# folkol/query-engines

Measured on AMD Instinct MI355X. Metric: rows/sec filter+project+group-by over 1B-row Arrow batch; % HBM roofline, higher is better.
Workload: dtype int64; 1 GPU; C4: SELECT k, SUM(a+b), COUNT(*), MIN(a), MAX(b) WHERE a > 2^19 GROUP BY k; rows_per_gpu=1000000000, groups=1024, columns=k, a, b int64 (Arrow, no nulls), parallelism=hash-sharded partial aggregate x1

## Files before the change

query-engines_amd/csrc/qe_dev.hpp:

```cpp
#ifndef QE_DEV_HPP
#define QE_DEV_HPP

#ifndef QE_OP_EQ
#define QE_OP_EQ 10
#define QE_OP_NE 11
#define QE_OP_LT 12
#define QE_OP_LE 13
#define QE_OP_GT 14
#define QE_OP_GE 15
#endif
#ifndef QE_MAX_KEYS
#define QE_MAX_KEYS 4
#define QE_MAX_AGGS 8
#define QE_MAX_COLS 8
#define QE_MAX_TERMS 8
#define QE_MAX_TOKENS 16
#endif
#ifndef QE_AGG_SUM
#define QE_AGG_SUM 1
#define QE_AGG_MIN 2
#define QE_AGG_MAX 3
#define QE_AGG_COUNT 4
#define QE_AGG_COUNT_STAR 5
#define QE_AGG_AVG 6
// ... 85 lines not shown
  const qu32* defer_in;
  qu32* defer_out;
  qu8* ovf;
  qu64 ovf_cap;
  qi32 ncols, nterms, mask_col, naggs;
  qi32 key_mode, nkeys, key_f64, rec_bytes;
  qi32 key_col[QE_MAX_KEYS], key_shift[QE_MAX_KEYS], key_nullbit[QE_MAX_KEYS], pad0;
  qi64 key_fmask[QE_MAX_KEYS];
  qi32 lds_log2, off_cstar;
  qi32 all8;
  qi32 nn_skip;
  qi32 off_acc[QE_MAX_AGGS], off_nn[QE_MAX_AGGS], off_idx[QE_MAX_AGGS];
  qu8* part_rec;
  qi64* part_off;
  qi64 part_tw;
  qi64* part_slice;
  qi64* part_chunk;
  qi32* part_sorted;
  qi32 mp_n, mp_pass;
  qi32 part_narrow;
  qi32 lds_compact;
  qu64 mp_keep;
  qu64* host_ctl;
};

__host__ __device__ inline qi64 f64_bits(double d) { return __builtin_bit_cast(qi64, d); }
__host__ __device__ inline double bits_f64(qi64 b) { return __builtin_bit_cast(double, b); }

__host__ __device__ inline qi64 f64_okey(double d) {
  const qi64 b = f64_bits(d == 0.0 ? 0.0 : d);
  return b >= 0 ? b : (b ^ 0x7FFFFFFFFFFFFFFFll);
}
__host__ __device__ inline double okey_f64(qi64 k) { return bits_f64(k >= 0 ? k : (k ^ 0x7FFFFFFFFFFFFFFFll)); }

__host__ __device__ inline qu64 fmix64(qu64 k) {
  k ^= k >> 33;
  k *= 0xFF51AFD7ED558CCDull;
  k ^= k >> 33;
  k *= 0xC4CEB9FE1A85EC53ull;
  k ^= k >> 33;
  return k;
}

__device__ inline qu32 spill_hash(qu64 key) {
  qu32 x = (qu32)key ^ (qu32)(key >> 32) * 0x27D4EB2Fu;
  x ^= x >> 16;
// ... 814 lines not shown
```

query-engines_amd/csrc/qe_hashagg.hip:

```cpp
#include <map>
#include <memory>
#include <mutex>

#include "qe_internal.hpp"

namespace qe {

constexpr int HA_THREADS = 512;
constexpr size_t HA_LDS_BUDGET = 80 * 1024;

__device__ __forceinline__ qi64* lds_keys(char* smem) { return (qi64*)smem; }

__device__ __forceinline__ void lds_init(const Plan& P, char* smem) {
  const int SS = (1 << P.lds_log2) + 2;
  qi64* keys = lds_keys(smem);
  qu32* cst = (qu32*)(smem + P.off_cstar);
  for (int s = threadIdx.x; s < SS; s += blockDim.x) {
    keys[s] = EMPTY_KEY;
    cst[s] = 0;
  }
#pragma unroll
  for (int j = 0; j < QE_MAX_AGGS; ++j) {
    if (j >= P.naggs) break;
    const DAgg& a = P.aggs[j];
    if (a.acc != ACC_NONE) {
// ... 1338 lines not shown
  size_t part_slc_bytes = 0;
  bool part_wide = false;
  bool narrow_failed = false;
  bool compact_off = false;
  uint8_t* ovf = nullptr;
  uint64_t ovf_cap = 0;
  uint32_t* defer[2] = {nullptr, nullptr};
  size_t defer_words = 0;
  bool defer_dirty[2] = {false, false};
  bool ctl_rows_clean = false;
  hipEvent_t ev[2] = {nullptr, nullptr};
  double last_kernel_ms = 0.0;
  int last_launches = 0;
  int last_specialized = 0;
  uint64_t last_sig = 0;
  std::string jit_note;
  bool async = false;
  bool pending = false;
  std::unique_ptr<qe::Plan> pend_plan;
  size_t pend_lds = 0;
  int pend_out_i = 0;
  uint64_t* ctl_pin = nullptr;
  hipEvent_t ev_ctl = nullptr;
  int poisoned = 0;
  std::string poison_msg;
  qe::Keyed* keyed = nullptr;
  int32_t flags = 0;
  uint64_t version = 0;
};

namespace qe {

int hashagg_expected_groups(const qe_hashagg* h, int64_t* out) {
  QE_CHECK(h && out, QE_ERR_INVALID_ARG, "null argument");
  *out = h->create_groups;
  return QE_OK;
}

qe_ctx* hashagg_ctx(const qe_hashagg* h) { return h ? h->ctx : nullptr; }

HashaggInfo hashagg_info(const qe_hashagg* h) {
  HashaggInfo I{};
  I.ctx = h->ctx;
  I.km = h->km;
  I.rec_bytes = h->rec_bytes;
  I.naggs = h->naggs;
// ... 581 lines not shown
    P.part_off = (qi64*)off;
    P.part_rec = h->part_rec;
    QE_TRY(jit_launch(ctx, fs, (int)g, P, sblock));
    QE_TRY(launch_check("qe_pscatter"));
  }
  const int64_t target = std::max<int64_t>((int64_t)1 << log2p, std::min<int64_t>((int64_t)ctx->num_cus * 8, R >> 15));
  const int64_t cw = std::max<int64_t>(256, (int64_t)div_up((uint64_t)std::max<int64_t>(R, 1) * 5, (uint64_t)target * 4));
  const int64_t max_slices = ((int64_t)1 << log2p) + (int64_t)div_up((uint64_t)std::max<int64_t>(R, 1), (uint64_t)cw);
  QE_TRY(grow_buffer(&h->part_slc, &h->part_slc_bytes, (size_t)(2 + 2 * max_slices) * 8, ctx, "partition slices"));
  hipLaunchKernelGGL(k_part_slices, dim3(1), dim3(1024), 0, ctx->stream, (const qi64*)off, (qi32)(1 << log2p), (qi64)g,
                     (qi64)cw, (qi64*)h->part_slc);
  QE_TRY(launch_check("k_part_slices"));
  P.n = R;
  P.part_tw = cw;
  P.part_rec = h->part_rec;
  P.part_slice = (qi64*)h->part_slc;
  *grid = (int)max_slices;
  h->jit_note = "radix-partitioned: " + std::to_string(1 << log2p) + " buckets, " + std::to_string(R) + " records of " +
                std::to_string(rb) + " B (" + (L.colmode ? "column" : "value") + (L.narrow ? " words, 32-bit)" : " words)") +
                (staged ? ", staged scatter" : "");
  return QE_OK;
}

static int launch_pass(qe_hashagg* h, Plan& P, size_t& lds, hipFunction_t pfn, int pgrid, int pass, int mp,
                       int out_i, const uint32_t* defer_in, int pblock = 0) {
  qe_ctx* ctx = h->ctx;
  const int64_t n = P.n;
  QE_CHECK(pass < 64, QE_ERR_CAPACITY, "hash aggregate did not converge after %d passes", pass);
  if (h->defer_dirty[out_i]) {
    QE_HIP(hipMemsetAsync(h->defer[out_i], 0, h->defer_words * 4, ctx->stream));
    h->defer_dirty[out_i] = false;
  }
  if (!h->ctl_rows_clean) QE_HIP(hipMemsetAsync(h->ctl + 1, 0, 16, ctx->stream));
  h->ctl_rows_clean = false;
  int32_t tracked = 0;
  for (int j = 0; j < P.naggs; ++j)
    if (P.aggs[j].track_nn) tracked |= 1 << j;
  QE_TRY(nn_materialize(h, tracked));
  P.nn_skip = h->nn_implicit;
  P.t = h->t;
  P.defer_in = defer_in;
  P.defer_out = h->defer[out_i];
  const int64_t waves = (int64_t)div_up((uint64_t)n, 256);
  const int per_cu = lds ? std::max<int>(1, std::min<int>(8, (int)((160 * 1024) / lds))) : 8;
  const int64_t gcap = std::min<int64_t>((int64_t)ctx->num_cus * per_cu, h->grid);
  int grid = (int)std::min<int64_t>((int64_t)div_up((uint64_t)waves, HA_THREADS / 64), gcap);
  if (grid < 1) grid = 1;
  hipFunction_t jfn = pfn;
  int jgrid = pgrid;
  if (pfn) {
  } else if (lds && ctx->jit) {
    static std::mutex memo_mu;
    static std::map<std::string, std::pair<hipFunction_t, int>> memo;
    const std::string key = plan_shape_key(ctx, P);
    int bpc = 0;
    bool have = false;
    {
      std::lock_guard<std::mutex> g(memo_mu);
      auto it = memo.find(key);
      if (it != memo.end()) {
        jfn = it->second.first;
        bpc = it->second.second;
        have = true;
      }
    }
    std::string src;
    size_t jl = 0;
    if (have || gen_fused_source(P, P.lds_log2, &src, &jl)) {
      if (have || jit_kernel(ctx, src, &jfn, &bpc, "qe_fused", fused_block(P.lds_log2)) == QE_OK) {
        if (!have) {
          std::lock_guard<std::mutex> g(memo_mu);
          memo[key] = {jfn, bpc};
        }
        static const int wg_env = [] {
          const char* e = getenv("QE_FUSED_WG_PER_CU");
          return e && *e ? std::max(1, atoi(e)) : 0;
        }();
        const int64_t per_state = wg_env ? (int64_t)ctx->num_cus * wg_env
                                         : std::max<int64_t>(ctx->num_cus, h->grid * 512 / fused_block(P.lds_log2));
        jgrid = (int)std::min<int64_t>(std::min<int64_t>((int64_t)ctx->num_cus * bpc, per_state),
                                       (int64_t)div_up((uint64_t)waves, fused_block(P.lds_log2) / 64));
        if (jgrid < 1) jgrid = 1;
        h->jit_note.clear();
        if (P.lds_compact) h->jit_note = "compact LDS table: " + std::to_string(P.lds_compact) + " slots";
      } else {
        h->jit_note = qe_last_error();
        jfn = nullptr;
      }
    } else {
      h->jit_note = "plan shape not specialisable";
    }
  } else if (h->jit_note.rfind("partitioning unavailable", 0) != 0) {
    h->jit_note = lds ? "jit disabled" : "global-only launch";
  }
  bool own_layout = false;
  for (int j = 0; j < h->naggs; ++j) own_layout = own_layout || h->acc[j] == ACC_SUM_X || P.aggs[j].share;
  if (!jfn && lds && (lds > HA_LDS_BUDGET || (own_layout && ctx->jit))) {
    size_t b = 0;
    int log2 = P.lds_log2;
    while (log2 >= h->lds_log2_min && (b = lds_layout_at(h, &P, log2, true)) > HA_LDS_BUDGET) --log2;
    if (log2 < h->lds_log2_min || log2 < 8) {
      P.lds_log2 = 0;
      lds = 0;
    } else {
      lds = b;
    }
    const int pc = lds ? std::max<int>(1, std::min<int>(8, (int)((160 * 1024) / lds))) : 8;
    grid = (int)std::max<int64_t>(1, std::min<int64_t>((int64_t)div_up((uint64_t)waves, HA_THREADS / 64),
                                                       std::min<int64_t>((int64_t)ctx->num_cus * pc, h->grid)));
  }
  if (!jfn) {
    const int pcu = lds ? std::max<int>(1, std::min<int>(2048 / HA_THREADS, (int)((160 * 1024) / lds))) : 2048 / HA_THREADS;
    h->jit_note += std::string(h->jit_note.empty() ? "" : "; ") + "generic kernel: " + std::to_string(lds / 1024) +
                   " KiB LDS table, " + std::to_string(pcu) + " workgroups per CU";
  }
  if (pass > 0 || mp > 0) QE_HIP(hipEventRecord(h->ev[0], ctx->stream));
  if (jfn) {
    QE_TRY(jit_launch(ctx, jfn, jgrid, P, pfn ? (pblock ? pblock : pagg_block()) : fused_block(P.lds_log2)));
  } else {
    QE_TRY(launch_hashagg(P, grid, lds, ctx->stream));
  }
  h->last_specialized = jfn ? 1 : 0;
  {
    const uint64_t k = jfn ? jit_kernel_signature(jfn) : 0x6E65726963ull;
    const uint64_t shape = jfn ? ((uint64_t)jgrid << 20) ^ (uint64_t)(pfn ? (pblock ? pblock : pagg_block()) : fused_block(P.lds_log2))
                               : ((uint64_t)grid << 20) ^ (uint64_t)lds;
    h->last_sig = fmix64(k ^ fmix64(shape));
  }
  QE_TRY(launch_check("k_hashagg"));
  QE_HIP(hipEventRecord(h->ev[1], ctx->stream));
  QE_HIP(hipMemcpyAsync(h->ctl_pin, h->ctl, 64, hipMemcpyDeviceToHost, ctx->stream));
  QE_HIP(hipEventRecord(h->ev_ctl, ctx->stream));
  return QE_OK;
}

static int settle_pass(qe_hashagg* h, const Plan& P, int* out_i, const uint32_t** defer_in, bool* done) {
  uint64_t c[8];
  QE_HIP(hipEventSynchronize(h->ev_ctl));
  memcpy(c, h->ctl_pin, 64);
  QE_CHECK((c[3] & CTL_KEY_TOO_LONG) == 0, QE_ERR_INVALID_ARG,
           "a UTF8 group key is longer than its column's max_len promised (qe_column.max_len)");
  QE_CHECK(c[3] == 0, QE_ERR_CAPACITY, "hash aggregate lost %llu groups (probe limit or overflow area)",
           (unsigned long long)c[3]);
  {
    float ms = 0.f;
    QE_HIP(hipEventElapsedTime(&ms, h->ev[0], h->ev[1]));
    h->last_kernel_ms += ms;
    h->last_launches += 1;
  }
  QE_CHECK(c[3] == 0, QE_ERR_CAPACITY, "hash aggregate lost %llu groups (overflow area)", (unsigned long long)c[3]);
  h->narrow_failed = P.part_narrow && (c[7] & 1) != 0;
  if (P.lds_compact && (c[7] & 2)) h->compact_off = true;
  const uint64_t groups = c[0], deferred = c[1], ovf_recs = std::min<uint64_t>(c[2], P.ovf_cap);
  h->ctl_rows_clean = c[1] == 0 && c[2] == 0;
  *done = true;
  if (deferred == 0 && ovf_recs == 0) {
    if (groups * 2 > h->t.cap) QE_TRY(table_grow(h, 4 * h->t.cap));
    h->known_groups = (int64_t)groups;
    return QE_OK;
  }
  QE_TRY(table_grow(h, std::max<uint64_t>(4 * h->t.cap, 2 * (groups + ovf_recs))));
  if (ovf_recs) QE_TRY(import_records(h, h->ovf, (int64_t)ovf_recs));
  if (deferred == 0) return QE_OK;
  h->defer_dirty[*out_i] = true;
  *defer_in = h->defer[*out_i];
  *out_i ^= 1;
  *done = false;
  return QE_OK;
}

static void adapt_after_update(qe_hashagg* h, size_t lds, int lds_log2) {
  if (h->known_groups > 0 && h->ctx->jit) {
// ... 147 lines not shown
    QE_TRY(settle_pass(h, Q, &out_i, &defer_in, &done));
    if (done) break;
  }
  h->jit_note = std::string("multi-pass: 2 buckets") + (P.lds_compact ? " (compact kept table)" : "") +
                ", bucket 1 spilled" + (SB > 1 ? " in " + std::to_string(SB) + " sub-buckets" : std::string()) + " as " +
                std::to_string(rb) + " B records (" + (L.colmode ? "column" : "value") + (L.narrow ? " words, 32-bit)" : " words)");
  return QE_OK;
}

static int run_update(qe_hashagg* h, Plan& P) {
  qe_ctx* ctx = h->ctx;
  QE_TRY(settle_pending(h));
  const int64_t rows = P.n;
  if (rows == 0) return QE_OK;
  size_t lds = lds_layout(h, &P);
  P.mp_n = 0;
  P.mp_pass = 0;
  P.ovf = h->ovf;
  P.ovf_cap = h->ovf_cap;
  QE_TRY(ensure_defer(h, rows));
  h->known_groups = -1;
  h->last_kernel_ms = 0.0;
  h->last_launches = 0;
  h->chunk_cap = 0;
  hipFunction_t pfn = nullptr;
  int pgrid = 0;
  QE_HIP(hipEventRecord(h->ev[0], ctx->stream));
  size_t lds_mp = 0;
  int mp_n = 0;
  const char* ce = getenv("QE_LDS_COMPACT");
  if (!lds && ctx->jit && h->expected_groups > 0 && !h->compact_off && !(ce && ce[0] == '0') && compact_ok(P)) {
    Plan T = P;
    T.lds_log2 = 16;
    const size_t bps = compact_slot_bytes(T);
    const int64_t nsl = ((int64_t)((lds_budget(ctx) - 512) / bps) - 66) & ~(int64_t)63;
    static const int cload = [] {
      const char* e = getenv("QE_COMPACT_LOAD");
      const int v = e && *e ? atoi(e) : 98;
      return v >= 50 && v <= 99 ? v : 98;
    }();
    if (nsl >= 512 && nsl * cload >= h->expected_groups * 100) {
      T.lds_compact = (qi32)nsl;
      std::string src;
      size_t jl = 0;
      hipFunction_t f = nullptr;
      int bpc = 0;
      if (gen_fused_source(T, T.lds_log2, &src, &jl) && jit_kernel(ctx, src, &f, &bpc, "qe_fused", fused_block(16)) == QE_OK) {
        const uint64_t need = (uint64_t)ctx->num_cus * 8 * ((uint64_t)nsl + 2);
        if (h->ovf_cap < need) {
          dev_free(ctx, h->ovf);
          h->ovf = nullptr;
          h->ovf_cap = 0;
          QE_TRY(dev_alloc(ctx, need * h->rec_bytes, (void**)&h->ovf));
// ... 287 lines not shown
    const qe_agg_desc& d = aggs[j];
    h->aggs[j] = d;
    const bool f = d.input_type == QE_TYPE_FLOAT64;
    const bool i = d.input_type == QE_TYPE_INT64 || d.input_type == QE_TYPE_INT32 ||
                   d.input_type == QE_TYPE_DATE32 || d.input_type == QE_TYPE_UINT8;
    if (d.fn != QE_AGG_COUNT_STAR && d.fn != QE_AGG_COUNT && !i && !f)
      return bail(fail(QE_ERR_UNSUPPORTED, "aggregate %d: input type %d (int64/int32/date32/uint8/fp64 only)", j,
                       d.input_type));
    switch (d.fn) {
      case QE_AGG_SUM: h->acc[j] = f ? (det ? ACC_SUM_X : ACC_SUM_F) : ACC_SUM_I; break;
      case QE_AGG_MIN: h->acc[j] = f ? ACC_MIN_F : ACC_MIN_I; break;
      case QE_AGG_MAX: h->acc[j] = f ? ACC_MAX_F : ACC_MAX_I; break;
      case QE_AGG_AVG: h->acc[j] = det ? ACC_SUM_X : ACC_SUM_F; break;
      case QE_AGG_COUNT:
      case QE_AGG_COUNT_STAR: h->acc[j] = ACC_NONE; break;
      default: return bail(fail(QE_ERR_UNSUPPORTED, "aggregate %d: unknown function %d", j, d.fn));
    }
    h->rec_bytes += agg_rec_bytes(h->acc[j]);
  }
  if (hipEventCreate(&h->ev[0]) != hipSuccess || hipEventCreate(&h->ev[1]) != hipSuccess ||
      hipEventCreateWithFlags(&h->ev_ctl, hipEventDisableTiming) != hipSuccess)
    return bail(fail(QE_ERR_DEVICE, "hipEventCreate failed"));
  if (pinned_slot_alloc(&h->ctl_pin) != QE_OK) return bail(QE_ERR_OOM);
  if (dev_alloc(ctx, 64, (void**)&h->ctl) != QE_OK) return bail(fail(QE_ERR_OOM, "control allocation failed"));
  const int64_t eg = expected_groups > 0 ? expected_groups : 1024;
  h->expected_groups = eg;
  h->create_groups = eg;
  int log2 = 8, log2_min = 8;
  while (log2 < 16 && ((int64_t)1 << log2) < 2 * eg) ++log2;
  while (log2_min < 16 && ((int64_t)1 << log2_min) < (5 * eg + 3) / 4) ++log2_min;
  const size_t budget = lds_budget(ctx);
  while (log2 > log2_min && lds_bytes_min(h, log2) > budget) --log2;
  h->lds_log2 = lds_bytes_min(h, log2) <= budget ? log2 : 0;
  h->lds_log2_min = log2_min;
  const int per_cu = h->lds_log2 ? std::max<int>(1, std::min<int>(8, (int)((160 * 1024) / lds_bytes_min(h, h->lds_log2)))) : 8;
  h->grid = ctx->num_cus * per_cu;
  if (h->lds_log2) {
    h->ovf_cap = (uint64_t)h->grid * (((uint64_t)1 << h->lds_log2) + 2);
    if (dev_alloc(ctx, h->ovf_cap * h->rec_bytes, (void**)&h->ovf) != QE_OK) {
      dev_free(ctx, h->ctl);
      return bail(fail(QE_ERR_OOM, "overflow area allocation failed"));
    }
  }
  const int st = table_alloc(h, std::max<uint64_t>(1024, next_pow2((uint64_t)(2 * eg))), &h->table_mem, &h->t, h->ctl);
  h->nn_implicit = all_nn_bits(h);
  if (st != QE_OK) {
    dev_free(ctx, h->ovf);
    dev_free(ctx, h->ctl);
    return bail(st);
  }
  h->ctl_rows_clean = true;
  *out = h;
  return QE_OK;
}

int qe_hashagg_destroy(qe_hashagg* h) {
  if (!h) return QE_OK;
  (void)hipSetDevice(h->ctx->device);
  qe_ctx* ctx = h->ctx;
  void* bufs[] = {h->table_mem, h->ctl, h->ovf, h->part_cnt, h->part_rec, h->part_slc, h->defer[0], h->defer[1]};
  for (void* b : bufs) dev_free(ctx, b);
  if (h->keyed) keyed_destroy(ctx, h->keyed);
  for (int i = 0; i < 2; ++i) {
    if (h->ev[i]) (void)hipEventDestroy(h->ev[i]);
  }
  if (h->ev_ctl) (void)hipEventDestroy(h->ev_ctl);
  pinned_slot_free(h->ctl_pin, ctx->stream);
  delete h;
  return QE_OK;
}

int qe_hashagg_last_kernel_kind(qe_hashagg* h, int32_t* specialized, char* note, int32_t note_len) {
  QE_CHECK(h && specialized, QE_ERR_INVALID_ARG, "null argument");
  *specialized = h->last_specialized;
  if (note && note_len > 0) {
    strncpy(note, h->jit_note.c_str(), (size_t)note_len - 1);
    note[note_len - 1] = 0;
  }
  return QE_OK;
}

int qe_hashagg_last_kernel_signature(qe_hashagg* h, uint64_t* sig) {
  QE_CHECK(h && sig, QE_ERR_INVALID_ARG, "null argument");
  *sig = h->last_sig;
  return QE_OK;
}

int qe_hashagg_last_kernel_time(qe_hashagg* h, double* ms, int32_t* launches) {
  QE_CHECK(h && ms, QE_ERR_INVALID_ARG, "null argument");
  QE_TRY(ctx_enter(h->ctx));
  QE_TRY(settle_pending(h));
  *ms = h->last_kernel_ms;
  if (launches) *launches = h->last_launches;
  return QE_OK;
}

int qe_hashagg_last_chunk_stats(qe_hashagg* h, int64_t* chunks, int64_t* full_chunks, int64_t* records) {
  QE_CHECK(h && chunks && full_chunks && records, QE_ERR_INVALID_ARG, "null argument");
  QE_TRY(ctx_enter(h->ctx));
  QE_TRY(settle_pending(h));
  *chunks = *full_chunks = *records = 0;
  if (h->chunk_cap <= 0 || !h->part_cnt) return QE_OK;
  QE_TRY(ctx_sync(h->ctx));
  int64_t ids = 0;
  QE_HIP(hipMemcpy(&ids, h->part_cnt, 8, hipMemcpyDeviceToHost));
  ids = std::max<int64_t>(0, std::min<int64_t>(ids, h->chunk_cap));
  std::vector<int64_t> meta((size_t)ids);
  if (ids) QE_HIP(hipMemcpy(meta.data(), h->part_cnt + 1, (size_t)ids * 8, hipMemcpyDeviceToHost));
  for (const int64_t w : meta) {
    if (w < 0) continue;
    const int64_t fill = w & 0xFFFFFFFFll;
    *chunks += 1;
    *full_chunks += fill == PART_CH ? 1 : 0;
    *records += fill;
  }
  return QE_OK;
}

int qe_hashagg_set_async(qe_hashagg* h, int32_t enable) {
  QE_CHECK(h, QE_ERR_INVALID_ARG, "null state");
  QE_TRY(ctx_enter(h->ctx));
  if (!enable) QE_TRY(settle_pending(h));
  h->async = enable != 0;
  return QE_OK;
}

int qe_hashagg_reset(qe_hashagg* h) {
  QE_CHECK(h, QE_ERR_INVALID_ARG, "null state");
  QE_TRY(ctx_enter(h->ctx));
  if (h->pending) {
    h->pending = false;
    h->defer_dirty[h->pend_out_i] = true;
  }
  h->poisoned = 0;
  h->poison_msg.clear();
  const int grid = (int)std::min<uint64_t>(div_up(h->t.cap + 2, 256), 4096);
  hipLaunchKernelGGL(k_table_init, dim3(grid), dim3(256), 0, h->ctx->stream, h->t, agg_meta(h), (qu64*)h->ctl, 1);
  QE_TRY(launch_check("k_table_init"));
  h->nn_implicit = all_nn_bits(h);
  h->ctl_rows_clean = true;
  h->row_base = 0;
  h->known_groups = 0;
  ++h->version;
  return QE_OK;
}

int qe_hashagg_set_row_base(qe_hashagg* h, int64_t row_base) {
  QE_CHECK(h && row_base >= 0, QE_ERR_INVALID_ARG, "bad arguments");
  h->row_base = row_base;
  return QE_OK;
}

static_assert(sizeof(Plan) <= 4096, "kernel argument must stay under 4 KiB");

int qe_hashagg_update_fused(qe_hashagg* h, const qe_column* cols, int32_t ncols, const qe_fused_spec* spec) {
  QE_CHECK(h && cols && spec, QE_ERR_INVALID_ARG, "null argument");
  QE_TRY(ctx_enter(h->ctx));
  if (keyed_dict(h->keyed)) return keyed_update_fused(h, cols, ncols, spec);
  return hashagg_update_fused_raw(h, cols, ncols, spec);
}

int qe_hashagg_update(qe_hashagg* h, const qe_column* keys, const qe_column* agg_inputs, const qe_column* mask) {
  QE_CHECK(h, QE_ERR_INVALID_ARG, "null state");
  QE_TRY(ctx_enter(h->ctx));
  QE_CHECK(h->nkeys == 0 || keys, QE_ERR_INVALID_ARG, "null keys");
  if (keyed_dict(h->keyed)) return keyed_update(h, keys, agg_inputs, mask);
  return hashagg_update_raw(h, keys, agg_inputs, mask);
}

}

namespace qe {

int hashagg_update_fused_raw(qe_hashagg* h, const qe_column* cols, int32_t ncols, const qe_fused_spec* spec) {
  Plan P;
  QE_TRY(compile_plan(h, cols, ncols, spec, &P));
  ++h->version;
  return run_update(h, P);
}

int hashagg_update_raw(qe_hashagg* h, const qe_column* keys, const qe_column* agg_inputs, const qe_column* mask) {
  QE_CHECK(h->naggs == 0 || agg_inputs, QE_ERR_INVALID_ARG, "null agg_inputs");
  qe_column cols[QE_MAX_COLS];
  int ncols = 0;
  int64_t n = -1;
  auto slot_of = [&](const qe_column& c, int* slot) -> int {
    if (n < 0) n = c.length;
    QE_CHECK(c.length == n, QE_ERR_INVALID_ARG, "input columns differ in length (%lld vs %lld)",
             (long long)c.length, (long long)n);
    for (int i = 0; i < ncols; ++i)
      if (cols[i].values == c.values && cols[i].validity == c.validity && cols[i].type == c.type) {
        *slot = i;
        return QE_OK;
      }
    QE_CHECK(ncols < QE_MAX_COLS, QE_ERR_UNSUPPORTED, "more than %d distinct input columns", QE_MAX_COLS);
    cols[ncols] = c;
    *slot = ncols++;
    return QE_OK;
  };
// ... 278 lines not shown
```

query-engines_amd/csrc/qe_internal.hpp:

```cpp
#pragma once

#include <hip/hip_runtime.h>
#include <stdint.h>
#include <string.h>

#include <algorithm>
#include <cmath>
#include <string>

#include "qe_hip.h"
#include "qe_dev.hpp"

struct qe_ctx {
  int device = 0;
  hipStream_t stream = nullptr;
  bool own_stream = false;
  int num_cus = 256;
  void* scratch = nullptr;
  size_t scratch_bytes = 0;
  uint64_t scratch_epoch = 0;
  void* pinned = nullptr;
  size_t pinned_bytes = 0;
  void* pinned_fg = nullptr;
  size_t pinned_fg_bytes = 0;
// ... 95 lines not shown
int hashagg_export_raw(qe_hashagg* h, int32_t nparts, void* dst);
int hashagg_export_counts_raw(qe_hashagg* h, int32_t nparts, int64_t* counts);
int hashagg_import_raw(qe_hashagg* h, const void* recs, int64_t nrec);
int hashagg_update_raw(qe_hashagg* h, const qe_column* dev_keys, const qe_column* agg_inputs, const qe_column* mask);
int hashagg_update_fused_raw(qe_hashagg* h, const qe_column* cols, int32_t ncols, const qe_fused_spec* spec);
int hashagg_finalize_raw(qe_hashagg* h, qe_column* dev_keys, qe_column* out_aggs, int64_t* out_groups, bool keys_only);
int keyed_create(qe_ctx* ctx, int32_t nkeys, const int32_t* types, int64_t expected, Keyed** out, int32_t* dev_nkeys,
                 int32_t* dev_types);
void keyed_destroy(qe_ctx* ctx, Keyed* K);
bool keyed_dict(const Keyed* K);
bool keyed_tuple(const Keyed* K);
int keyed_update(qe_hashagg* h, const qe_column* keys, const qe_column* agg_inputs, const qe_column* mask);
int keyed_update_fused(qe_hashagg* h, const qe_column* cols, int32_t ncols, const qe_fused_spec* spec);
int keyed_finalize(qe_hashagg* h, qe_column* out_keys, qe_column* out_aggs, int64_t* out_groups);
int strdict_encode_packed_checked(qe_ctx* ctx, const qe_column* in, qe_column* codes, unsigned long long* err);
constexpr uint64_t CTL_KEY_TOO_LONG = 1ull << 62;
bool gen_pscatter_staged_source(const qe::Plan& P, int log2p, std::string* src, bool chunked = false, bool soa = false);
bool part_static();
bool part_soa();
int jit_kernel(qe_ctx* ctx, const std::string& src, hipFunction_t* fn, int* blocks_per_cu,
               const char* name = "qe_fused", int block = 512);
int jit_launch(qe_ctx* ctx, hipFunction_t fn, int grid, const qe::Plan& P, int block = 512);
std::string plan_shape_key(const qe_ctx* ctx, const qe::Plan& P);
int compile_inputs(const qe_column* cols, int32_t ncols, int32_t mask_col, int32_t nterms, const qe_pred_term* terms,
                   qe::Plan* P, bool* col_f64);
int compile_program(const qe_column* cols, int32_t ncols, const bool* col_f64, const qe_agg_program& pg, int j,
                    qe::DAgg* a, bool* is_f, bool* nullable);
enum { SP_COUNTER = 0, SP_PERSIST = 1, SP_COUNT = 2, SP_WRITE = 3, SP_WRITE_SCAN = 4, SP_RESIDENT = 5 };
int selproj_resident_rows(const qe::Plan& P, const int32_t* out_kind, int nout, int64_t n, int cus);
bool gen_selproj_resident_source(const qe::Plan& P, const int32_t* out_kind, int nout, int R, std::string* src);
bool gen_selproj_source(const qe::Plan& P, const int32_t* out_kind, int nout, std::string* src, int mode);
int selproj_block(int mode);
int selproj_rows_per_thread(const qe::Plan& P, int mode);
uint64_t jit_kernel_signature(hipFunction_t fn);
bool selproj_pipelined();
int selproj_rows(const qe::Plan& P, int mode);
bool selproj_nt(const qe::Plan& P);
int exclusive_scan_i64(qe_ctx* ctx, const int64_t* in, int64_t* out, int64_t n);
int64_t utf8_gather_tiles(int64_t rows);
int utf8_gather_lengths(qe_ctx* ctx, const int2* sl, int64_t rows, int64_t* tsum);
int utf8_gather_copy(qe_ctx* ctx, const int2* sl, int64_t rows, const int64_t* tsum, const uint8_t* src,
                     int32_t* out_offs, uint8_t* out_values);

inline int type_width(int32_t t) {
  switch (t) {
    case QE_TYPE_INT64:
// ... 86 lines not shown
```

query-engines_amd/csrc/qe_jit.hip:

```cpp
#include <hip/hiprtc.h>
#include <stdio.h>
#include <stdlib.h>
#include <fcntl.h>
#include <string.h>
#include <sys/stat.h>
#include <unistd.h>

#include <map>
#include <mutex>
#include <sstream>
#include <vector>

#include "qe_internal.hpp"

namespace qe {

static const char* kDevHeader =
#include "qe_dev.inc"
    ;

namespace {

struct Expr {
  std::string v;
// ... 73 lines not shown

std::string acc_init(int acc) {
  switch (acc) {
    case ACC_MIN_I:
    case ACC_MIN_F: return "0x7FFFFFFFFFFFFFFFll";
    case ACC_MAX_I:
    case ACC_MAX_F: return "EMPTY_KEY";
    default: return "0";
  }
}

bool use_nt() {
  const char* e = getenv("QE_NT");
  return !(e && e[0] == '0');
}
}

bool fused_prefetch() {
  static const bool v = [] {
    const char* e = getenv("QE_FUSED_PF");
    return e && e[0] == '1';
  }();
  return v;
}
int fused_block(int lds_log2) {
  (void)lds_log2;
  static const int env = [] {
    const char* e = getenv("QE_FUSED_BLOCK");
    const int b = e ? atoi(e) : 0;
    return (b == 256 || b == 512 || b == 1024) ? b : 0;
  }();
  return env ? env : 1024;
}

namespace {

std::string ld(const std::string& type, const std::string& ptr, bool nt = true) {
  if (nt && use_nt()) return "__builtin_nontemporal_load((const " + type + "*)(" + ptr + "))";
  return "(*(const " + type + "*)(" + ptr + "))";
}

void emit_predicate(const Plan& P, std::ostringstream& o, int rows) {
  const std::string loop = "#pragma unroll\n    for (int r = 0; r < " + std::to_string(rows) + "; ++r) ";
  if (P.mask_col >= 0) {
    o << loop << "if (!((qu32)(" << col_raw(P.mask_col) << " & 1) & " << col_ok(P, P.mask_col)
      << ")) act &= ~(1u << r);\n";
// ... 532 lines not shown
    if (P.aggs[j].acc != ACC_NONE) b += compact_acc32(P, j) ? 4 : 8;
    if (P.aggs[j].track_nn) b += 4;
  }
  return b;
}

bool gen_fused_source(const Plan& P, int log2, std::string* src, size_t* lds_bytes, bool spill) {
  if (log2 < 4 || log2 > 16 || P.ncols < 1 || P.ncols > QE_MAX_COLS) return false;
  if (spill && P.mp_n < 2) return false;
  const bool compact = P.lds_compact > 0;
  if (compact && !compact_ok(P)) return false;
  std::vector<Expr> ex;
  if (!agg_inputs(P, &ex)) return false;
  std::vector<std::string> val(P.naggs), ok(P.naggs);
  for (int j = 0; j < P.naggs; ++j) {
    val[j] = ex[j].v;
    ok[j] = ex[j].ok;
  }
  std::ostringstream o;
  const bool pf = fused_prefetch();
  o << "\nusing namespace qe;\n"
    << "extern \"C\" __global__ void __launch_bounds__(" << fused_block(log2) << ") qe_fused(const Plan P) {\n"
    << "  __shared__ qu32 s_newg;\n  if (threadIdx.x == 0) s_newg = 0;\n";
  const int SB = spill ? P.mp_n - 1 : 0;
  if (spill && (SB & (SB - 1))) return false;
  if (spill)
    o << "  constexpr int SB = " << SB << ";\n  qi64 sp_cid[SB];\n  qu32 sp_fill[SB];\n"
      << "#pragma unroll\n  for (int b = 0; b < SB; ++b) { sp_cid[b] = -1; sp_fill[b] = 0; }\n  qu32 nfit = 0;\n";
  if (compact) emit_lds_table_c(P, o, lds_bytes);
  else emit_lds_table(P, o, log2, lds_bytes);
  const int block = fused_block(log2);
  const bool fxq = !compact && !spill && P.mp_n <= 1 && fx_queue_enabled() && !fx_queue_aggs(P).empty() &&
                   fx_queue_aggs(P).size() <= 8 && (1 << log2) + 2 < (1 << 24) &&
                   *lds_bytes + fx_queue_bytes(P, block) <= (size_t)152 * 1024;
  if (fxq) {
    emit_fx_queue_decl(P, o, block);
    *lds_bytes += fx_queue_bytes(P, block);
  }
  o << "  const int lane = threadIdx.x & 63;\n"
    << "  const qi64 wave = (blockIdx.x * (qi64)blockDim.x + threadIdx.x) >> 6;\n"
    << "  const qi64 stride = (((qi64)gridDim.x * blockDim.x) >> 6) * 256;\n";
  if (pf) {
    o << "  {\n    const qi64 base = wave * 256;\n    const bool full = base + 256 <= P.n;\n"
      << "    const qi64 r0 = base + 2 * lane;\n";
    emit_col_loads(P, o, ~0u, "p", true);
    o << "  for (qi64 base = wave * 256; base < P.n; base += stride) {\n"
// ... 84 lines not shown
      << "            const qu64 pos = k < room ? (qu64)sp_cid[b] * PART_CH + sp_fill[b] + k : (qu64)nid * PART_CH + (k - room);\n"
      << "            qi64 w[" << L.words << "];\n";
    emit_record_words(P, L, ex, "w", o);
    emit_fit_check(L, "w", o);
    const char* wt = L.narrow ? "qi32" : "qi64";
    o << "            " << wt << "* const dst = (" << wt << "*)(P.part_rec + pos * " << RB << "ull);\n";
    for (int q = 0; q < L.words; ++q) o << "            dst[" << q << "] = (" << wt << ")w[" << q << "];\n";
    o << "          }\n          kb += (qu32)__popcll(bal[r]);\n        }\n"
      << "        sp_cid[b] = nid;\n        sp_fill[b] = tot - room;\n"
      << "      }\n    }\n"
      << "    if (act == 0) continue;\n";
  } else if (P.mp_n > 1)
    o << "#pragma unroll\n    for (int r = 0; r < 4; ++r)\n"
      << "      if (((act >> r) & 1) && (P.mp_pass < 0 ? spill_hash((qu64)key[r]) < P.mp_keep\n"
      << "                                              : (qu32)__umul64hi(fmix64((qu64)key[r]), (qu64)P.mp_n) != (qu32)P.mp_pass))\n"
      << "        act &= ~(1u << r);\n"
      << "    if (act == 0) continue;\n";
  if (compact)
    emit_agg_rows_c(P, o, val, ok, "P.row_base + r0 + 128 * (r >> 1) + (r & 1)", "r0 + 128 * (r >> 1) + (r & 1)");
  else
    emit_agg_rows(P, o, val, ok, "P.row_base + r0 + 128 * (r >> 1) + (r & 1)", "r0 + 128 * (r >> 1) + (r & 1)", fxq,
                  log2 <= 8);
  o << (pf ? "    } while (0);\n  }\n  }\n" : "  }\n");
  if (fxq) {
    o << "  if (q_n) {\n";
    emit_fx_queue_run(P, o, "q_n");
    o << "  }\n";
  }
  if (spill)
    o << "#pragma unroll\n  for (int b = 0; b < SB; ++b)\n"
      << "    if ((threadIdx.x & 63) == 0 && sp_cid[b] >= 0) P.part_chunk[1 + sp_cid[b]] = ((qi64)b << 32) | (qi64)sp_fill[b];\n"
      << "  if (nfit) atomicOr(&P.t.ctl[7], 1ull);\n";
  if (compact) emit_flush_c(P, o);
  else emit_flush(P, o);
  o << "  __syncthreads();\n  if (threadIdx.x == 0 && s_newg) atomicAdd(&P.t.ctl[0], (qu64)s_newg);\n}\n";
  static const bool fx_inline = [] {
    const char* e = getenv("QE_FX_INLINE");
    return !(e && e[0] == '0');
  }();
  *src = std::string(fx_inline ? "#define QE_FX_INLINE 1\n" : "") + kDevHeader + o.str();
  return true;
}

PartLayout part_layout(const Plan& P) {
  PartLayout L{};
  bool knull = false, vnull = false, cnull = false;
  for (int k = 0; k < P.nkeys; ++k) knull = knull || P.cols[P.key_col[k]].valid != nullptr;
  int nv = 0;
  unsigned cm = 0;
  for (int j = 0; j < P.naggs; ++j) {
    if (P.aggs[j].pkind == 0) continue;
    ++nv;
    vnull = vnull || P.aggs[j].track_nn;
    L.row = L.row || acc_is_f64mm(P.aggs[j].acc);
    for (int t = 0; t < P.aggs[j].ntok; ++t)
      if (P.aggs[j].tok[t].op == T_COL) cm |= 1u << P.aggs[j].tok[t].arg;
  }
  for (int c = 0; c < P.ncols; ++c)
// ... 962 lines not shown
            : "      const qi64* rp = (const qi64*)(P.part_rec + i * " + std::to_string(8 * L.words) + "ull);\n")
    << "      const qi64 k = rp[0];\n";
  if (L.flags_word >= 0)
    o << "      const bool kn = rp[" << L.flags_word << (soa ? " * PART_CH" : "") << "] & 1;\n";
  else
    o << "      const bool kn = false;\n";
  o << "      int s = kn ? S : (k == EMPTY_KEY ? S + 1 : -1);\n"
    << "      if (s < 0) { const qu32 hh = lds_hash((qu64)k) >> (32 - LOG2); s = s_keys[hh] == k ? (int)hh : lds_probe(s_keys, LOG2, k, hh); }\n"
    << "      if (s >= 0 && (s_cst[s] & 0x80000000u)) {\n"
    << "        atomicOr((qu32*)&P.defer_out[i >> 5], 1u << (i & 31));\n"
    << "        atomicAdd(&P.t.ctl[1], 1ull);\n      }\n    }\n  }\n"
    << "  if (threadIdx.x == 0 && s_newg) atomicAdd(&P.t.ctl[0], (qu64)s_newg);\n";
  o << "}\n";
  *src = std::string(kDevHeader) + o.str();
  return true;
}

bool selproj_nt(const Plan& P) {
  const char* e = getenv("QE_SELPROJ_NT");
  if (e && *e) return e[0] == '1';
  return P.n > (64ll << 20);
}

std::string plan_shape_key(const qe_ctx* ctx, const Plan& P) {
  Plan k;
  memset(&k, 0, sizeof k);
  memcpy(&k, &P, sizeof P);
  for (int c = 0; c < QE_MAX_COLS; ++c) {
    k.cols[c].p = (const void*)(uintptr_t)(P.cols[c].p != nullptr);
    k.cols[c].valid = (const qu8*)(uintptr_t)(P.cols[c].valid != nullptr);
  }
  for (int t = 0; t < QE_MAX_TERMS; ++t) k.terms[t].lit = 0;
  for (int j = 0; j < QE_MAX_AGGS; ++j) {
    k.aggs[j].rhs_lit = 0;
    for (int t = 0; t < QE_MAX_TOKENS; ++t) k.aggs[j].tok[t].lit = 0;
  }
  memset(&k.t, 0, sizeof k.t);
  k.n = k.row_base = 0;
  k.defer_in = nullptr;
  k.defer_out = nullptr;
  k.ovf = nullptr;
  k.ovf_cap = 0;
  k.part_rec = nullptr;
  k.part_off = nullptr;
  k.part_tw = 0;
  k.part_slice = nullptr;
  k.part_chunk = nullptr;
  k.part_sorted = nullptr;
  k.mp_keep = 0;
  k.host_ctl = nullptr;
  const int32_t extra[2] = {ctx->device, use_nt() ? 1 : 0};
  return std::string((const char*)&k, sizeof k) + std::string((const char*)extra, sizeof extra);
}

int selproj_block(int mode) {
  static const int all = [] {
    const char* e = getenv("QE_SELPROJ_BLOCK");
    const int b = e && *e ? atoi(e) : 0;
    return (b == 256 || b == 512 || b == 1024) ? b : 0;
  }();
  static const int lb = [] {
    const char* e = getenv("QE_SELPROJ_LB_BLOCK");
    const int b = e && *e ? atoi(e) : 1024;
    return (b == 256 || b == 512) ? b : 1024;
  }();
  if (all) return all;
  return (mode == SP_PERSIST || mode == SP_COUNTER) ? lb : 256;
}

int selproj_lbw() {
  static const int v = [] {
    const char* e = getenv("QE_SELPROJ_LBW");
    const int k = e && *e ? atoi(e) : 1;
// ... 748 lines not shown
```

Baseline: 271.7 billion rows/s.

## Publish fused-kernel counters to pinned host memory and memoize plan and shape lookups

The last workgroup of the fused kernel, picked by an atomic ticket, now writes the control counters straight into pinned host memory along with a sequence number. The host spin-waits on that sequence number instead of issuing a D2H memcpy and waiting on an event, and reading the kernel's elapsed time is deferred until it is requested. Compiled plans and JIT shape-key lookups are also memoized per handle, which skips compile_plan and the string key/map lookup on repeated calls. The cost is a ticket atomic and a vmcnt wait at kernel end, plus host CPU spinning. Optional per-workgroup timestamps can be enabled through an env var for profiling.

After: 276.3 billion rows/s (median of 6 runs). +1.7%, better.

```diff
diff --git a/query-engines_amd/csrc/qe_dev.hpp b/query-engines_amd/csrc/qe_dev.hpp
--- a/query-engines_amd/csrc/qe_dev.hpp
+++ b/query-engines_amd/csrc/qe_dev.hpp
@@ -131,6 +131,8 @@
   qi32 lds_compact;
   qu64 mp_keep;
   qu64* host_ctl;
+  qu64 host_seq;
+  qu64* stamps;
 };
 
 __host__ __device__ inline qi64 f64_bits(double d) { return __builtin_bit_cast(qi64, d); }
diff --git a/query-engines_amd/csrc/qe_hashagg.hip b/query-engines_amd/csrc/qe_hashagg.hip
--- a/query-engines_amd/csrc/qe_hashagg.hip
+++ b/query-engines_amd/csrc/qe_hashagg.hip
@@ -1,6 +1,10 @@
+#include <atomic>
+#include <chrono>
+#include <cstdio>
 #include <map>
 #include <memory>
 #include <mutex>
+#include <vector>
 
 #include "qe_internal.hpp"
 
@@ -1385,6 +1389,25 @@
   int pend_out_i = 0;
   uint64_t* ctl_pin = nullptr;
   hipEvent_t ev_ctl = nullptr;
+  uint64_t pub_seq = 0;
+  bool time_pending = false;
+  struct PlanMemo {
+    qe_fused_spec spec;
+    int32_t ncols = 0;
+    int32_t type[QE_MAX_COLS] = {};
+    bool nullable[QE_MAX_COLS] = {};
+    qe::Plan P;
+  };
+  std::unique_ptr<PlanMemo> plan_memo;
+  struct ShapeMemo {
+    qe::Plan k;
+    hipFunction_t fn = nullptr;
+    int bpc = 0;
+  };
+  std::unique_ptr<ShapeMemo> shape_memo;
+  uint64_t* stamps = nullptr;
+  size_t stamps_bytes = 0;
+  int stamps_wgs = 0;
   int poisoned = 0;
   std::string poison_msg;
   qe::Keyed* keyed = nullptr;
@@ -2012,6 +2035,62 @@
   return QE_OK;
 }
 
+static uint64_t next_publish_seq() {
+  static std::atomic<uint64_t> seq{0};
+  return seq.fetch_add(1, std::memory_order_relaxed) + 1;
+}
+
+static int resolve_kernel_time(qe_hashagg* h) {
+  if (!h->time_pending) return QE_OK;
+  h->time_pending = false;
+  float ms = 0.f;
+  hipError_t e = hipEventElapsedTime(&ms, h->ev[0], h->ev[1]);
+  if (e == hipErrorNotReady) {
+    (void)hipGetLastError();
+    QE_HIP(hipEventSynchronize(h->ev[1]));
+    e = hipEventElapsedTime(&ms, h->ev[0], h->ev[1]);
+  }
+  QE_HIP(e);
+  h->last_kernel_ms += ms;
+  if (h->stamps_wgs) {
+    std::vector<uint64_t> w(2 + 3 * (size_t)h->stamps_wgs);
+    w[0] = (uint64_t)h->stamps_wgs;
+    const double dms = ms;
+    memcpy(&w[1], &dms, 8);
+    QE_HIP(hipMemcpy(w.data() + 2, h->stamps, (w.size() - 2) * 8, hipMemcpyDeviceToHost));
+    h->stamps_wgs = 0;
+    FILE* f = fopen(fused_stamps_file(), "ab");
+    QE_CHECK(f != nullptr, QE_ERR_INVALID_ARG, "QE_FUSED_STAMPS: cannot open %s", fused_stamps_file());
+    const size_t put = fwrite(w.data(), 8, w.size(), f);
+    fclose(f);
+    QE_CHECK(put == w.size(), QE_ERR_DEVICE, "QE_FUSED_STAMPS: short write to %s", fused_stamps_file());
+  }
+  return QE_OK;
+}
+
+static int wait_published(qe_hashagg* h, uint64_t seq, uint64_t c[8]) {
+  volatile uint64_t* pv = h->ctl_pin;
+  auto t0 = std::chrono::steady_clock::now();
+  for (uint32_t i = 1; pv[6] != seq; ++i) {
+#if defined(__x86_64__) && !defined(__HIP_DEVICE_COMPILE__)
+    __builtin_ia32_pause();
+#endif
+    if ((i & 63) != 0) continue;
+    if (std::chrono::steady_clock::now() - t0 < std::chrono::microseconds(50)) continue;
+    t0 = std::chrono::steady_clock::now();
+    const hipError_t e = hipEventQuery(h->ev[1]);
+    if (e == hipSuccess) {
+      if (pv[6] != seq) return fail(QE_ERR_DEVICE, "hash aggregate kernel finished without publishing its counters");
+      break;
+    }
+    if (e != hipErrorNotReady) return fail(QE_ERR_DEVICE, "hash aggregate kernel failed: %s", hipGetErrorString(e));
+    (void)hipGetLastError();
+  }
+  std::atomic_thread_fence(std::memory_order_acquire);
+  for (int i = 0; i < 8; ++i) c[i] = pv[i];
+  return QE_OK;
+}
+
 static int launch_pass(qe_hashagg* h, Plan& P, size_t& lds, hipFunction_t pfn, int pgrid, int pass, int mp,
                        int out_i, const uint32_t* defer_in, int pblock = 0) {
   qe_ctx* ctx = h->ctx;
@@ -2042,10 +2121,18 @@
   } else if (lds && ctx->jit) {
     static std::mutex memo_mu;
     static std::map<std::string, std::pair<hipFunction_t, int>> memo;
-    const std::string key = plan_shape_key(ctx, P);
+    Plan shape;
+    plan_shape_mask(P, &shape);
     int bpc = 0;
     bool have = false;
-    {
+    const bool same = h->shape_memo && memcmp(&h->shape_memo->k, &shape, sizeof shape) == 0;
+    if (same) {
+      jfn = h->shape_memo->fn;
+      bpc = h->shape_memo->bpc;
+      have = true;
+    }
+    const std::string key = same ? std::string() : plan_shape_key(ctx, P);
+    if (!same) {
       std::lock_guard<std::mutex> g(memo_mu);
       auto it = memo.find(key);
       if (it != memo.end()) {
@@ -2061,6 +2148,12 @@
         if (!have) {
           std::lock_guard<std::mutex> g(memo_mu);
           memo[key] = {jfn, bpc};
+        }
+        if (!same) {
+          if (!h->shape_memo) h->shape_memo.reset(new qe_hashagg::ShapeMemo());
+          h->shape_memo->k = shape;
+          h->shape_memo->fn = jfn;
+          h->shape_memo->bpc = bpc;
         }
         static const int wg_env = [] {
           const char* e = getenv("QE_FUSED_WG_PER_CU");
@@ -2104,7 +2197,19 @@
     h->jit_note += std::string(h->jit_note.empty() ? "" : "; ") + "generic kernel: " + std::to_string(lds / 1024) +
                    " KiB LDS table, " + std::to_string(pcu) + " workgroups per CU";
   }
+  QE_TRY(resolve_kernel_time(h));
   if (pass > 0 || mp > 0) QE_HIP(hipEventRecord(h->ev[0], ctx->stream));
+  const bool publish = jfn && !pfn && pass == 0 && mp == 0 && P.mp_n == 0;
+  P.host_ctl = publish ? (qu64*)h->ctl_pin : nullptr;
+  P.host_seq = publish ? next_publish_seq() : 0;
+  h->pub_seq = P.host_seq;
+  P.stamps = nullptr;
+  h->stamps_wgs = 0;
+  if (publish && fused_stamps_file()) {
+    QE_TRY(grow_buffer(&h->stamps, &h->stamps_bytes, (size_t)jgrid * 24, ctx, "stamps"));
+    P.stamps = (qu64*)h->stamps;
+    h->stamps_wgs = jgrid;
+  }
   if (jfn) {
     QE_TRY(jit_launch(ctx, jfn, jgrid, P, pfn ? (pblock ? pblock : pagg_block()) : fused_block(P.lds_log2)));
   } else {
@@ -2119,6 +2224,7 @@
   }
   QE_TRY(launch_check("k_hashagg"));
   QE_HIP(hipEventRecord(h->ev[1], ctx->stream));
+  if (publish) return QE_OK;
   QE_HIP(hipMemcpyAsync(h->ctl_pin, h->ctl, 64, hipMemcpyDeviceToHost, ctx->stream));
   QE_HIP(hipEventRecord(h->ev_ctl, ctx->stream));
   return QE_OK;
@@ -2126,18 +2232,26 @@
 
 static int settle_pass(qe_hashagg* h, const Plan& P, int* out_i, const uint32_t** defer_in, bool* done) {
   uint64_t c[8];
-  QE_HIP(hipEventSynchronize(h->ev_ctl));
-  memcpy(c, h->ctl_pin, 64);
+  const uint64_t seq = h->pub_seq;
+  h->pub_seq = 0;
+  if (seq) {
+    QE_TRY(wait_published(h, seq, c));
+  } else {
+    QE_HIP(hipEventSynchronize(h->ev_ctl));
+    memcpy(c, h->ctl_pin, 64);
+  }
   QE_CHECK((c[3] & CTL_KEY_TOO_LONG) == 0, QE_ERR_INVALID_ARG,
            "a UTF8 group key is longer than its column's max_len promised (qe_column.max_len)");
   QE_CHECK(c[3] == 0, QE_ERR_CAPACITY, "hash aggregate lost %llu groups (probe limit or overflow area)",
            (unsigned long long)c[3]);
-  {
+  if (seq) {
+    h->time_pending = true;
+  } else {
     float ms = 0.f;
     QE_HIP(hipEventElapsedTime(&ms, h->ev[0], h->ev[1]));
     h->last_kernel_ms += ms;
-    h->last_launches += 1;
-  }
+  }
+  h->last_launches += 1;
   QE_CHECK(c[3] == 0, QE_ERR_CAPACITY, "hash aggregate lost %llu groups (overflow area)", (unsigned long long)c[3]);
   h->narrow_failed = P.part_narrow && (c[7] & 1) != 0;
   if (P.lds_compact && (c[7] & 2)) h->compact_off = true;
@@ -2331,13 +2445,14 @@
   h->known_groups = -1;
   h->last_kernel_ms = 0.0;
   h->last_launches = 0;
+  h->time_pending = false;
   h->chunk_cap = 0;
   hipFunction_t pfn = nullptr;
   int pgrid = 0;
   QE_HIP(hipEventRecord(h->ev[0], ctx->stream));
   size_t lds_mp = 0;
   int mp_n = 0;
-  const char* ce = getenv("QE_LDS_COMPACT");
+  const char* ce = !lds && ctx->jit ? getenv("QE_LDS_COMPACT") : nullptr;
   if (!lds && ctx->jit && h->expected_groups > 0 && !h->compact_off && !(ce && ce[0] == '0') && compact_ok(P)) {
     Plan T = P;
     T.lds_log2 = 16;
@@ -2671,6 +2786,7 @@
       hipEventCreateWithFlags(&h->ev_ctl, hipEventDisableTiming) != hipSuccess)
     return bail(fail(QE_ERR_DEVICE, "hipEventCreate failed"));
   if (pinned_slot_alloc(&h->ctl_pin) != QE_OK) return bail(QE_ERR_OOM);
+  h->ctl_pin[6] = 0;
   if (dev_alloc(ctx, 64, (void**)&h->ctl) != QE_OK) return bail(fail(QE_ERR_OOM, "control allocation failed"));
   const int64_t eg = expected_groups > 0 ? expected_groups : 1024;
   h->expected_groups = eg;
@@ -2707,7 +2823,8 @@
   if (!h) return QE_OK;
   (void)hipSetDevice(h->ctx->device);
   qe_ctx* ctx = h->ctx;
-  void* bufs[] = {h->table_mem, h->ctl, h->ovf, h->part_cnt, h->part_rec, h->part_slc, h->defer[0], h->defer[1]};
+  void* bufs[] = {h->table_mem, h->ctl, h->ovf, h->part_cnt, h->part_rec, h->part_slc, h->defer[0], h->defer[1],
+                  h->stamps};
   for (void* b : bufs) dev_free(ctx, b);
   if (h->keyed) keyed_destroy(ctx, h->keyed);
   for (int i = 0; i < 2; ++i) {
@@ -2739,6 +2856,7 @@
   QE_CHECK(h && ms, QE_ERR_INVALID_ARG, "null argument");
   QE_TRY(ctx_enter(h->ctx));
   QE_TRY(settle_pending(h));
+  QE_TRY(resolve_kernel_time(h));
   *ms = h->last_kernel_ms;
   if (launches) *launches = h->last_launches;
   return QE_OK;
@@ -2780,6 +2898,7 @@
   if (h->pending) {
     h->pending = false;
     h->defer_dirty[h->pend_out_i] = true;
+    h->pub_seq = 0;
   }
   h->poisoned = 0;
   h->poison_msg.clear();
@@ -2821,9 +2940,39 @@
 
 namespace qe {
 
+static bool plan_memo_hit(qe_hashagg* h, const qe_column* cols, int32_t ncols, const qe_fused_spec* spec, Plan* P) {
+  const qe_hashagg::PlanMemo* m = h->plan_memo.get();
+  if (!m || ncols < 1 || m->ncols != ncols || memcmp(&m->spec, spec, sizeof *spec) != 0) return false;
+  const int64_t n = cols[0].length;
+  for (int c = 0; c < ncols; ++c)
+    if (cols[c].type != m->type[c] || (cols[c].validity != nullptr) != m->nullable[c] || cols[c].length != n ||
+        !(cols[c].values || n == 0))
+      return false;
+  *P = m->P;
+  for (int c = 0; c < ncols; ++c) {
+    P->cols[c].p = cols[c].values;
+    P->cols[c].valid = cols[c].validity;
+  }
+  P->n = n;
+  P->row_base = h->row_base;
+  return true;
+}
+
 int hashagg_update_fused_raw(qe_hashagg* h, const qe_column* cols, int32_t ncols, const qe_fused_spec* spec) {
   Plan P;
-  QE_TRY(compile_plan(h, cols, ncols, spec, &P));
+  if (!plan_memo_hit(h, cols, ncols, spec, &P)) {
+    if (!h->plan_memo) h->plan_memo.reset(new qe_hashagg::PlanMemo());
+    qe_hashagg::PlanMemo* m = h->plan_memo.get();
+    m->ncols = -1;
+    QE_TRY(compile_plan(h, cols, ncols, spec, &P));
+    m->spec = *spec;
+    for (int c = 0; c < ncols; ++c) {
+      m->type[c] = cols[c].type;
+      m->nullable[c] = cols[c].validity != nullptr;
+    }
+    m->P = P;
+    m->ncols = ncols;
+  }
   ++h->version;
   return run_update(h, P);
 }
diff --git a/query-engines_amd/csrc/qe_internal.hpp b/query-engines_amd/csrc/qe_internal.hpp
--- a/query-engines_amd/csrc/qe_internal.hpp
+++ b/query-engines_amd/csrc/qe_internal.hpp
@@ -141,6 +141,8 @@
                const char* name = "qe_fused", int block = 512);
 int jit_launch(qe_ctx* ctx, hipFunction_t fn, int grid, const qe::Plan& P, int block = 512);
 std::string plan_shape_key(const qe_ctx* ctx, const qe::Plan& P);
+void plan_shape_mask(const qe::Plan& P, qe::Plan* out);
+const char* fused_stamps_file();
 int compile_inputs(const qe_column* cols, int32_t ncols, int32_t mask_col, int32_t nterms, const qe_pred_term* terms,
                    qe::Plan* P, bool* col_f64);
 int compile_program(const qe_column* cols, int32_t ncols, const bool* col_f64, const qe_agg_program& pg, int j,
diff --git a/query-engines_amd/csrc/qe_jit.hip b/query-engines_amd/csrc/qe_jit.hip
--- a/query-engines_amd/csrc/qe_jit.hip
+++ b/query-engines_amd/csrc/qe_jit.hip
@@ -119,6 +119,13 @@
     return e && e[0] == '1';
   }();
   return v;
+}
+const char* fused_stamps_file() {
+  static const std::string v = [] {
+    const char* e = getenv("QE_FUSED_STAMPS");
+    return std::string(e ? e : "");
+  }();
+  return v.empty() ? nullptr : v.c_str();
 }
 int fused_block(int lds_log2) {
   (void)lds_log2;
@@ -697,6 +704,12 @@
   o << "\nusing namespace qe;\n"
     << "extern \"C\" __global__ void __launch_bounds__(" << fused_block(log2) << ") qe_fused(const Plan P) {\n"
     << "  __shared__ qu32 s_newg;\n  if (threadIdx.x == 0) s_newg = 0;\n";
+  const bool stamps = !spill && fused_stamps_file() != nullptr;
+  auto stamp = [&](int w) {
+    if (stamps)
+      o << "  if (P.stamps && threadIdx.x == 0) P.stamps[3 * blockIdx.x + " << w << "] = __builtin_amdgcn_s_memrealtime();\n";
+  };
+  stamp(0);
   const int SB = spill ? P.mp_n - 1 : 0;
   if (spill && (SB & (SB - 1))) return false;
   if (spill)
@@ -827,6 +840,7 @@
     emit_agg_rows(P, o, val, ok, "P.row_base + r0 + 128 * (r >> 1) + (r & 1)", "r0 + 128 * (r >> 1) + (r & 1)", fxq,
                   log2 <= 8);
   o << (pf ? "    } while (0);\n  }\n  }\n" : "  }\n");
+  stamp(1);
   if (fxq) {
     o << "  if (q_n) {\n";
     emit_fx_queue_run(P, o, "q_n");
@@ -838,7 +852,27 @@
       << "  if (nfit) atomicOr(&P.t.ctl[7], 1ull);\n";
   if (compact) emit_flush_c(P, o);
   else emit_flush(P, o);
-  o << "  __syncthreads();\n  if (threadIdx.x == 0 && s_newg) atomicAdd(&P.t.ctl[0], (qu64)s_newg);\n}\n";
+  if (spill) {
+    o << "  __syncthreads();\n  if (threadIdx.x == 0 && s_newg) atomicAdd(&P.t.ctl[0], (qu64)s_newg);\n}\n";
+  } else {
+    o << "  if (P.host_ctl) asm volatile(\"s_waitcnt vmcnt(0)\" ::: \"memory\");\n"
+      << "  __syncthreads();\n";
+    stamp(2);
+    o << "  if (threadIdx.x == 0) {\n"
+      << "    if (s_newg) atomicAdd(&P.t.ctl[0], (qu64)s_newg);\n"
+      << "    if (P.host_ctl) {\n"
+      << "      __builtin_amdgcn_fence(__ATOMIC_RELEASE, \"agent\");\n"
+      << "      const qu64 tk = __hip_atomic_fetch_add(&P.t.ctl[6], 1ull, __ATOMIC_RELAXED, __HIP_MEMORY_SCOPE_AGENT);\n"
+      << "      if (tk == (qu64)gridDim.x - 1) {\n"
+      << "        __builtin_amdgcn_fence(__ATOMIC_ACQUIRE, \"agent\");\n"
+      << "        qu64 c[8];\n"
+      << "#pragma unroll\n        for (int i = 0; i < 8; ++i) c[i] = __hip_atomic_load(&P.t.ctl[i], __ATOMIC_RELAXED, __HIP_MEMORY_SCOPE_AGENT);\n"
+      << "#pragma unroll\n        for (int i = 0; i < 8; ++i) if (i != 6) P.host_ctl[i] = c[i];\n"
+      << "        __hip_atomic_store(&P.t.ctl[6], 0ull, __ATOMIC_RELAXED, __HIP_MEMORY_SCOPE_AGENT);  // the next launch's ticket\n"
+      << "        __builtin_amdgcn_fence(__ATOMIC_RELEASE, \"\");\n"
+      << "        __hip_atomic_store(&P.host_ctl[6], P.host_seq, __ATOMIC_RELAXED, __HIP_MEMORY_SCOPE_SYSTEM);\n"
+      << "      }\n    }\n  }\n}\n";
+  }
   static const bool fx_inline = [] {
     const char* e = getenv("QE_FX_INLINE");
     return !(e && e[0] == '0');
@@ -1847,9 +1881,8 @@
   return P.n > (64ll << 20);
 }
 
-std::string plan_shape_key(const qe_ctx* ctx, const Plan& P) {
-  Plan k;
-  memset(&k, 0, sizeof k);
+void plan_shape_mask(const Plan& P, Plan* out) {
+  Plan& k = *out;
   memcpy(&k, &P, sizeof P);
   for (int c = 0; c < QE_MAX_COLS; ++c) {
     k.cols[c].p = (const void*)(uintptr_t)(P.cols[c].p != nullptr);
@@ -1874,6 +1907,13 @@
   k.part_sorted = nullptr;
   k.mp_keep = 0;
   k.host_ctl = nullptr;
+  k.host_seq = 0;
+  k.stamps = nullptr;
+}
+
+std::string plan_shape_key(const qe_ctx* ctx, const Plan& P) {
+  Plan k;
+  plan_shape_mask(P, &k);
   const int32_t extra[2] = {ctx->device, use_nt() ? 1 : 0};
   return std::string((const char*)&k, sizeof k) + std::string((const char*)extra, sizeof extra);
 }
```
